# zhaihongjia/SplatLoc

Measured on AMD Instinct MI355X. Metric: fwd+bwd frames/s @1080p, 500k Gaussians, 32 feat-ch; HBM GB/s vs roofline, higher is better.
Workload: dtype f32

## Files before the change

### splatloc_amd/csrc/binning.hip

```cpp
#include "tile_order.h"
#include "composite_common.h"

namespace sr {

__device__ __forceinline__ int f2i_sat_b(float v)
{
    if (!(v > -1.0e9f)) v = -1.0e9f;
    if (!(v < 1.0e9f)) v = 1.0e9f;
    return (int)v;
}

constexpr int EMIT_BLOCK = 256;
constexpr int EMIT_IPT = 4;
static_assert(EMIT_SPAN == EMIT_BLOCK * EMIT_IPT, "common.h: EMIT_SPAN");

template <typename KeyT>
__global__ void __launch_bounds__(EMIT_BLOCK)
emit_kernel(int64_t R, int P , int Pv , int tiles_per_view, int W, int H,
            const uint32_t* __restrict__ offsets,
            const uint32_t* __restrict__ depth_order, const float4* __restrict__ rec,
            KeyT* __restrict__ keys, uint32_t* __restrict__ vals,
            const uint32_t* __restrict__ span_owner ,
            uint32_t* __restrict__ ranges, uint32_t nranges )
{
    for (uint32_t w = blockIdx.x * blockDim.x + threadIdx.x; w < nranges; w += gridDim.x * blockDim.x) ranges[w] = 0u;
    __shared__ uint32_t s_off[EMIT_SPAN + 1];
    __shared__ uint32_t s_gid[EMIT_SPAN], s_org[EMIT_SPAN], s_w[EMIT_SPAN];
    __shared__ int s_min;
    const int t = threadIdx.x;
    const int64_t j0 = (int64_t)blockIdx.x * EMIT_SPAN;
    const uint32_t j0u = (uint32_t)j0;
    int lo = 0, hi = P;
    if (span_owner && blockIdx.x < SPAN_OWNER_CAP) {
        lo = (int)span_owner[blockIdx.x];
        hi = lo + 1;
    }
    while (hi - lo > 1) {
        const int n = hi - lo;
        const int step = (n + EMIT_BLOCK - 1) / EMIT_BLOCK;
        if (t == 0) s_min = EMIT_BLOCK;
        __syncthreads();
        const int last = lo + (t + 1) * step - 1;
        if (last >= hi - 1 || offsets[last] > j0u) atomicMin(&s_min, t);
        __syncthreads();
        const int seg = s_min;
        __syncthreads();
        lo = lo + seg * step;
        hi = min(hi, lo + step);
    }
    const int r_lo = lo;
    for (int q = t; q <= EMIT_SPAN; q += EMIT_BLOCK) {
        const int r = r_lo - 1 + q;
        s_off[q] = r < 0 ? 0u : offsets[min(r, P - 1)];
    }
    __syncthreads();
    const int gx = (W + TILE - 1) / TILE, gy = (H + TILE - 1) / TILE;
    const uint32_t j_last = (uint32_t)(min(R, j0 + (int64_t)EMIT_SPAN) - 1);
    int nr;
    {
        int a = 1, b = EMIT_SPAN + 1;
        while (a < b) {
            const int mid = (a + b) >> 1;
            if (s_off[mid] > j_last) b = mid; else a = mid + 1;
        }
        nr = a;
    }
    for (int q = t; q < nr; q += EMIT_BLOCK) {
        const uint32_t g = depth_order[r_lo + q] & 0xFFFFFFu;
        const float4 p = rec[2 * g];
        const float rf = p.w;
        const int rminx = min(gx, max(0, f2i_sat_b((p.x - rf) / (float)TILE)));
        const int rminy = min(gy, max(0, f2i_sat_b((p.y - rf) / (float)TILE)));
        const int rmaxx = min(gx, max(0, f2i_sat_b((p.x + rf + (float)(TILE - 1)) / (float)TILE)));
        s_gid[q] = g;
        const uint32_t v = (P == Pv) ? 0u : g / (uint32_t)Pv;
        s_org[q] = v * (uint32_t)tiles_per_view + (uint32_t)rminy * (uint32_t)gx + (uint32_t)rminx;
        s_w[q] = (uint32_t)(rmaxx - rminx);
    }
    __syncthreads();
#pragma unroll
    for (int it = 0; it < EMIT_IPT; ++it) {
        const int64_t j = j0 + it * EMIT_BLOCK + t;
        if (j < R) {
            const uint32_t ju = (uint32_t)j;
            int a = 1, b = nr + 1;
            while (a < b) {
                const int mid = (a + b) >> 1;
                if (s_off[mid] > ju) b = mid; else a = mid + 1;
            }
            const uint32_t k = ju - s_off[a - 1];
            const uint32_t w = s_w[a - 1];
            const uint32_t row = k / w;
            keys[j] = (KeyT)(s_org[a - 1] + row * (uint32_t)gx + (k - row * w));
            vals[j] = s_gid[a - 1];
        }
    }
}

int launch_emit(const FramePlan& p, int64_t R, const GeomView& g, uint32_t* keys, uint32_t* vals, uint32_t* ranges,
                uint32_t nranges, hipStream_t stream, bool keys16)
{
    if (R == 0) return SPLATRASTER_OK;
    const int64_t blocks = (R + EMIT_SPAN - 1) / EMIT_SPAN;
    const int n = p.P * p.V;
    const uint32_t* owner = scan_state_bytes(n) ? g.span_owner : nullptr;
    if (keys16)
        hipLaunchKernelGGL(emit_kernel<uint16_t>, dim3((unsigned)blocks), dim3(EMIT_BLOCK), 0, stream, R, n, p.P, p.tiles, p.W, p.H,
                           g.offsets, g.depth_order, g.rec, reinterpret_cast<uint16_t*>(keys), vals, owner, ranges, nranges);
    else
        hipLaunchKernelGGL(emit_kernel<uint32_t>, dim3((unsigned)blocks), dim3(EMIT_BLOCK), 0, stream, R, n, p.P, p.tiles, p.W, p.H,
                           g.offsets, g.depth_order, g.rec, keys, vals, owner, ranges, nranges);
    SR_LAUNCH_CHECK();
    return SPLATRASTER_OK;
}

int launch_ranges_clear(int32_t tiles, uint32_t* ranges, hipStream_t stream)
{
    SR_HIP_CHECK(hipMemsetAsync(ranges, 0, sizeof(uint32_t) * 2 * (size_t)tiles, stream));
    return SPLATRASTER_OK;
}

#ifndef SR_PAYLOAD_NT_MIN
#define SR_PAYLOAD_NT_MIN (8ll << 20)
#endif
static int64_t g_payload_stream_min = SR_PAYLOAD_NT_MIN;
void set_payload_stream_min(int64_t instances) { g_payload_stream_min = instances < 0 ? (int64_t)SR_PAYLOAD_NT_MIN : instances; }

template <bool NT>
__global__ void __launch_bounds__(256)
payload_kernel(int64_t R, int gx, int tiles_per_view, int V, const uint32_t* __restrict__ point_list,
               const uint32_t* __restrict__ tile_list, const float4* __restrict__ rec,
               float4* __restrict__ irec, uint32_t* __restrict__ ipack, uint32_t* __restrict__ ranges)
{
    const int64_t j = (int64_t)blockIdx.x * blockDim.x + threadIdx.x;
    if (j >= R) return;
    const uint32_t g = point_list[j], t = tile_list[j];
    const float4 a0 = rec[2 * (size_t)g], a1 = rec[2 * (size_t)g + 1];
    uint32_t tl = t;
#pragma unroll 1
    for (int v = 1; v < V && tl >= (uint32_t)tiles_per_view; ++v) tl -= (uint32_t)tiles_per_view;
    const uint32_t ty = tl / (uint32_t)gx, tx = tl - ty * (uint32_t)gx;
    const float4 c1 = payload_conic(a1);
    const uint32_t m = g | (quadrant_reach_mask(a0, a1, (float)(tx * TILE), (float)(ty * TILE)) << 24);
    if (NT) {
        typedef float f32x4_t __attribute__((ext_vector_type(4)));
        f32x4_t* out = reinterpret_cast<f32x4_t*>(irec) + 2 * j;
        __builtin_nontemporal_store((f32x4_t){a0.x, a0.y, a0.z, a0.w}, out);
        __builtin_nontemporal_store((f32x4_t){c1.x, c1.y, c1.z, c1.w}, out + 1);
        __builtin_nontemporal_store(m, ipack + j);
    } else {
        irec[2 * j] = a0;
        irec[2 * j + 1] = c1;
        ipack[j] = m;
    }
    if (j == 0 || tile_list[j - 1] != t) ranges[2 * t] = (uint32_t)j;
    if (j == R - 1 || tile_list[j + 1] != t) ranges[2 * t + 1] = (uint32_t)(j + 1);
}

int launch_payload(const FramePlan& p, int64_t R, const GeomView& g, const BinView& b, hipStream_t stream)
{
    if (R == 0) return SPLATRASTER_OK;
    if (R >= g_payload_stream_min)
        hipLaunchKernelGGL(payload_kernel<true>, dim3((unsigned)((R + 255) / 256)), dim3(256), 0, stream, R, p.gx, p.tiles, p.V,
                           b.point_list, b.tile_list, g.rec, b.irec, b.ipack, b.ranges);
    else
        hipLaunchKernelGGL(payload_kernel<false>, dim3((unsigned)((R + 255) / 256)), dim3(256), 0, stream, R, p.gx, p.tiles, p.V,
                           b.point_list, b.tile_list, g.rec, b.irec, b.ipack, b.ranges);
    SR_LAUNCH_CHECK();
    return SPLATRASTER_OK;
}

__global__ void __launch_bounds__(256)
ranges_kernel(int64_t R, const uint32_t* __restrict__ tile_list, uint32_t* __restrict__ ranges)
{
    const int64_t j = (int64_t)blockIdx.x * blockDim.x + threadIdx.x;
    if (j >= R) return;
    const uint32_t t = tile_list[j];
    if (j == 0 || tile_list[j - 1] != t) ranges[2 * t] = (uint32_t)j;
    if (j == R - 1 || tile_list[j + 1] != t) ranges[2 * t + 1] = (uint32_t)(j + 1);
}

template <bool NT>
__global__ void __launch_bounds__(256)
payload_tile_kernel(int gx, int tiles_per_view, const uint32_t* __restrict__ ranges, const uint32_t* __restrict__ point_list,
                    const float4* __restrict__ rec, float4* __restrict__ irec, uint32_t* __restrict__ ipack,
                    uint32_t* __restrict__ cranges)
{
    __shared__ uint32_t s_live[4];
    const uint32_t gt = blockIdx.x;
    const uint32_t beg = ranges[2 * gt], end = ranges[2 * gt + 1];
    const uint32_t tl = gt % (uint32_t)tiles_per_view;
    const uint32_t ty = tl / (uint32_t)gx, tx = tl - ty * (uint32_t)gx;
    const float ox = (float)(tx * TILE), oy = (float)(ty * TILE);
    const int lane = threadIdx.x & (WAVE - 1);
    const int wave = __builtin_amdgcn_readfirstlane((int)(threadIdx.x >> 6));
    const uint64_t lt_mask = (lane == 0) ? 0ull : (~0ull >> (WAVE - lane));
    uint32_t running = 0;
#pragma unroll 1
    for (uint32_t base = beg; base < end; base += 256u) {
        const uint32_t j = base + threadIdx.x;
        uint32_t g = 0u, mask = 0u;
        float4 a0 = make_float4(0.f, 0.f, 0.f, 0.f), a1 = a0;
        if (j < end) {
            g = point_list[j];
            a0 = rec[2 * (size_t)g];
            a1 = rec[2 * (size_t)g + 1];
            mask = quadrant_reach_mask(a0, a1, ox, oy);
        }
        const bool live = mask != 0u;
        const uint64_t ballot = __builtin_amdgcn_ballot_w64(live);
        if (lane == 0) s_live[wave] = (uint32_t)__popcll(ballot);
        __syncthreads();
        const uint32_t n0 = s_live[0], n1 = s_live[1], n2 = s_live[2], n3 = s_live[3];
        __syncthreads();
        const uint32_t before = (wave > 0 ? n0 : 0u) + (wave > 1 ? n1 : 0u) + (wave > 2 ? n2 : 0u);
        if (live) {
            const size_t pos = (size_t)beg + running + before + (uint32_t)__popcll(ballot & lt_mask);
            const float4 c1 = payload_conic(a1);
            const float back = __uint_as_float(j - beg + 1u);
            const uint32_t m = g | (mask << 24);
            if (NT) {
                typedef float f32x4_t __attribute__((ext_vector_type(4)));
                f32x4_t* out = reinterpret_cast<f32x4_t*>(irec) + 2 * pos;
                __builtin_nontemporal_store((f32x4_t){a0.x, a0.y, a0.z, back}, out);
                __builtin_nontemporal_store((f32x4_t){c1.x, c1.y, c1.z, c1.w}, out + 1);
                __builtin_nontemporal_store(m, ipack + pos);
            } else {
                irec[2 * pos] = make_float4(a0.x, a0.y, a0.z, back);
                irec[2 * pos + 1] = c1;
                ipack[pos] = m;
            }
        }
        running += n0 + n1 + n2 + n3;
    }
    if (threadIdx.x == 0) {
        cranges[2 * gt] = beg;
        cranges[2 * gt + 1] = beg + running;
    }
}

int launch_payload_compact(const FramePlan& p, int64_t R, const GeomView& g, const BinView& b, uint32_t* cranges, hipStream_t stream)
{
    const unsigned lists = (unsigned)p.gtiles;
    if (R > 0) {
        hipLaunchKernelGGL(ranges_kernel, dim3((unsigned)((R + 255) / 256)), dim3(256), 0, stream, R, b.tile_list, b.ranges);
        SR_LAUNCH_CHECK();
    }
    if (R >= g_payload_stream_min)
        hipLaunchKernelGGL(payload_tile_kernel<true>, dim3(lists), dim3(256), 0, stream, p.gx, p.tiles, b.ranges, b.point_list, g.rec,
                           b.irec, b.ipack, cranges);
    else
        hipLaunchKernelGGL(payload_tile_kernel<false>, dim3(lists), dim3(256), 0, stream, p.gx, p.tiles, b.ranges, b.point_list, g.rec,
                           b.irec, b.ipack, cranges);
    SR_LAUNCH_CHECK();
    return SPLATRASTER_OK;
}

__global__ void __launch_bounds__(ORDER_THREADS)
tile_order_kernel(int T, const uint32_t* __restrict__ ranges, uint32_t* __restrict__ order, uint32_t* __restrict__ nparts)
{
    __shared__ uint32_t s_cnt[ORDER_BUCKETS];
    __shared__ uint32_t s_wsum[ORDER_THREADS / WAVE];
    tile_order_block(T, [&](int i) { return ranges[2 * i + 1] - ranges[2 * i]; }, order, s_cnt, s_wsum, nparts);
}

int launch_tile_order(const FramePlan& p, const BinView& b, hipStream_t stream)
{
    if (!p.order) return SPLATRASTER_OK;
    hipLaunchKernelGGL(tile_order_kernel, dim3(1), dim3(ORDER_THREADS), 0, stream, (int)p.gtiles, b.ranges, b.tile_order, b.nparts);
    SR_LAUNCH_CHECK();
    return SPLATRASTER_OK;
}

__global__ void __launch_bounds__(256)
pad_features_kernel(int64_t n4 , int C, int PPR, const float* __restrict__ feat,
                    float4* __restrict__ featp4)
{
    const int64_t e = (int64_t)blockIdx.x * blockDim.x + threadIdx.x;
    if (e >= n4) return;
    const int64_t row = e / PPR;
    const int c = (int)(e - row * PPR) * 4;
    const float* src = feat + row * C + c;
    float4 v;
    v.x = src[0];
    v.y = c + 1 < C ? src[1] : 0.0f;
    v.z = c + 2 < C ? src[2] : 0.0f;
    v.w = c + 3 < C ? src[3] : 0.0f;
    featp4[e] = v;
}

int launch_pad_features(int32_t P, int C, const float* feat, float* featp, hipStream_t stream)
{
    const int CP = padded_channels(C);
    const int64_t n4 = (int64_t)P * CP / 4;
    if (n4 == 0 || CP == C) return SPLATRASTER_OK;
    hipLaunchKernelGGL(pad_features_kernel, dim3((unsigned)((n4 + 255) / 256)), dim3(256), 0, stream, n4, C, CP / 4,
                       feat, reinterpret_cast<float4*>(featp));
    SR_LAUNCH_CHECK();
    return SPLATRASTER_OK;
}

}
```

Measured before the change: 766.6.

## Replace emit binary search with owner scan; vectorize ranges and pair rec loads

In the emit kernel, each span start marks its owning Gaussian in shared memory, and a wave-level max-scan with a carry across iterations propagates the owner to every slot. This replaces the per-element binary search, and the integer divide is swapped for a float reciprocal with a correction step. The ranges kernel now handles four tile ids per thread using aligned uint4 loads with a head offset. The payload compaction kernel has lane pairs fetch the two halves of two records and exchange them through DPP quad permutes, so each load instruction is coalesced. These changes add extra shared memory, synchronisation and tricky edge handling, which brings some correctness risk.

```diff
diff --git a/splatloc_amd/csrc/binning.hip b/splatloc_amd/csrc/binning.hip
--- a/splatloc_amd/csrc/binning.hip
+++ b/splatloc_amd/csrc/binning.hip
@@ -26,6 +26,8 @@
     for (uint32_t w = blockIdx.x * blockDim.x + threadIdx.x; w < nranges; w += gridDim.x * blockDim.x) ranges[w] = 0u;
     __shared__ uint32_t s_off[EMIT_SPAN + 1];
     __shared__ uint32_t s_gid[EMIT_SPAN], s_org[EMIT_SPAN], s_w[EMIT_SPAN];
+    __shared__ __attribute__((aligned(8))) uint16_t s_own[EMIT_SPAN];
+    __shared__ uint32_t s_wown[EMIT_BLOCK / WAVE];
     __shared__ int s_min;
     const int t = threadIdx.x;
     const int64_t j0 = (int64_t)blockIdx.x * EMIT_SPAN;
@@ -53,6 +55,7 @@
         const int r = r_lo - 1 + q;
         s_off[q] = r < 0 ? 0u : offsets[min(r, P - 1)];
     }
+    reinterpret_cast<uint2*>(s_own)[t] = make_uint2(0u, 0u);
     __syncthreads();
     const int gx = (W + TILE - 1) / TILE, gy = (H + TILE - 1) / TILE;
     const uint32_t j_last = (uint32_t)(min(R, j0 + (int64_t)EMIT_SPAN) - 1);
@@ -76,23 +79,42 @@
         const uint32_t v = (P == Pv) ? 0u : g / (uint32_t)Pv;
         s_org[q] = v * (uint32_t)tiles_per_view + (uint32_t)rminy * (uint32_t)gx + (uint32_t)rminx;
         s_w[q] = (uint32_t)(rmaxx - rminx);
+        if (q >= 1 && s_off[q + 1] > s_off[q]) s_own[s_off[q] - j0u] = (uint16_t)q;
     }
     __syncthreads();
+    {
+        const int lane = t & (WAVE - 1);
+        const uint2 ow = reinterpret_cast<const uint2*>(s_own)[t];
+        const uint32_t m0 = ow.x & 0xFFFFu, m1 = max(m0, ow.x >> 16), m2 = max(m1, ow.y & 0xFFFFu), m3 = max(m2, ow.y >> 16);
+        uint32_t incl = m3;
+#pragma unroll
+        for (int d = 1; d < WAVE; d <<= 1) {
+            const uint32_t up = (uint32_t)__shfl_up((int)incl, d, WAVE);
+            if (lane >= d) incl = max(incl, up);
+        }
+        uint32_t excl = (uint32_t)__shfl_up((int)incl, 1, WAVE);
+        if (lane == 0) excl = 0u;
+        if (lane == WAVE - 1) s_wown[t / WAVE] = incl;
+        reinterpret_cast<uint2*>(s_own)[t] = make_uint2(max(m0, excl) | max(m1, excl) << 16, max(m2, excl) | max(m3, excl) << 16);
+    }
+    __syncthreads();
+    uint32_t carry = 0u;
+    static_assert(WAVE * EMIT_IPT == EMIT_BLOCK && EMIT_BLOCK / WAVE == EMIT_IPT, "emit_kernel: a wave scans the slots of one iteration");
 #pragma unroll
     for (int it = 0; it < EMIT_IPT; ++it) {
         const int64_t j = j0 + it * EMIT_BLOCK + t;
+        const uint32_t a = max((uint32_t)s_own[it * EMIT_BLOCK + t], carry);
+        carry = max(carry, s_wown[it]);
         if (j < R) {
             const uint32_t ju = (uint32_t)j;
-            int a = 1, b = nr + 1;
-            while (a < b) {
-                const int mid = (a + b) >> 1;
-                if (s_off[mid] > ju) b = mid; else a = mid + 1;
-            }
-            const uint32_t k = ju - s_off[a - 1];
-            const uint32_t w = s_w[a - 1];
-            const uint32_t row = k / w;
-            keys[j] = (KeyT)(s_org[a - 1] + row * (uint32_t)gx + (k - row * w));
-            vals[j] = s_gid[a - 1];
+            const uint32_t k = ju - s_off[a];
+            const uint32_t w = s_w[a];
+            uint32_t row = (uint32_t)((float)k * __frcp_rn((float)w));
+            int col = (int)(k - row * w);
+            if (col < 0) { row -= 1u; col += (int)w; }
+            else if (col >= (int)w) { row += 1u; col -= (int)w; }
+            keys[j] = (KeyT)(s_org[a] + row * (uint32_t)gx + (uint32_t)col);
+            vals[j] = s_gid[a];
         }
     }
 }
@@ -171,13 +193,41 @@
 }
 
 __global__ void __launch_bounds__(256)
-ranges_kernel(int64_t R, const uint32_t* __restrict__ tile_list, uint32_t* __restrict__ ranges)
-{
-    const int64_t j = (int64_t)blockIdx.x * blockDim.x + threadIdx.x;
-    if (j >= R) return;
-    const uint32_t t = tile_list[j];
-    if (j == 0 || tile_list[j - 1] != t) ranges[2 * t] = (uint32_t)j;
-    if (j == R - 1 || tile_list[j + 1] != t) ranges[2 * t + 1] = (uint32_t)(j + 1);
+ranges_kernel(int64_t R, int head, const uint32_t* __restrict__ tile_list, uint32_t* __restrict__ ranges)
+{
+    const int64_t j0 = ((int64_t)blockIdx.x * blockDim.x + threadIdx.x) * 4 - head;
+    if (j0 >= R) return;
+    uint32_t t[6];
+    if (j0 >= 0 && j0 + 4 <= R) {
+        const uint4 q = *reinterpret_cast<const uint4*>(tile_list + j0);
+        t[1] = q.x; t[2] = q.y; t[3] = q.z; t[4] = q.w;
+        t[0] = j0 > 0 ? tile_list[j0 - 1] : 0u;
+        t[5] = j0 + 4 < R ? tile_list[j0 + 4] : 0u;
+    } else {
+#pragma unroll
+        for (int e = 0; e < 6; ++e) {
+            const int64_t j = j0 - 1 + e;
+            t[e] = (j >= 0 && j < R) ? tile_list[j] : 0u;
+        }
+    }
+#pragma unroll
+    for (int e = 1; e <= 4; ++e) {
+        const int64_t j = j0 - 1 + e;
+        if (j < 0 || j >= R) continue;
+        if (j == 0 || t[e - 1] != t[e]) ranges[2 * t[e]] = (uint32_t)j;
+        if (j == R - 1 || t[e + 1] != t[e]) ranges[2 * t[e] + 1] = (uint32_t)(j + 1);
+    }
+}
+
+template <int CTRL>
+__device__ __forceinline__ uint32_t quad_perm_u32(uint32_t v)
+{
+    return (uint32_t)__builtin_amdgcn_update_dpp(0, (int)v, CTRL, 0xf, 0xf, false);
+}
+__device__ __forceinline__ float4 quad_perm_f4(const float4& v)
+{
+    return make_float4(__uint_as_float(quad_perm_u32<0xB1>(__float_as_uint(v.x))), __uint_as_float(quad_perm_u32<0xB1>(__float_as_uint(v.y))),
+                       __uint_as_float(quad_perm_u32<0xB1>(__float_as_uint(v.z))), __uint_as_float(quad_perm_u32<0xB1>(__float_as_uint(v.w))));
 }
 
 template <bool NT>
@@ -195,18 +245,19 @@
     const int lane = threadIdx.x & (WAVE - 1);
     const int wave = __builtin_amdgcn_readfirstlane((int)(threadIdx.x >> 6));
     const uint64_t lt_mask = (lane == 0) ? 0ull : (~0ull >> (WAVE - lane));
+    const bool odd = threadIdx.x & 1u;
     uint32_t running = 0;
 #pragma unroll 1
     for (uint32_t base = beg; base < end; base += 256u) {
         const uint32_t j = base + threadIdx.x;
-        uint32_t g = 0u, mask = 0u;
-        float4 a0 = make_float4(0.f, 0.f, 0.f, 0.f), a1 = a0;
-        if (j < end) {
-            g = point_list[j];
-            a0 = rec[2 * (size_t)g];
-            a1 = rec[2 * (size_t)g + 1];
-            mask = quadrant_reach_mask(a0, a1, ox, oy);
-        }
+        const bool valid = j < end;
+        const uint32_t g = point_list[valid ? j : end - 1u];
+        const uint32_t ge = quad_perm_u32<0xA0>(g), go = quad_perm_u32<0xF5>(g);
+        const float4 x = rec[2 * (size_t)ge + odd];
+        const float4 y = rec[2 * (size_t)go + odd];
+        const float4 got = quad_perm_f4(odd ? x : y);
+        const float4 a0 = odd ? got : x, a1 = odd ? y : got;
+        const uint32_t mask = valid ? quadrant_reach_mask(a0, a1, ox, oy) : 0u;
         const bool live = mask != 0u;
         const uint64_t ballot = __builtin_amdgcn_ballot_w64(live);
         if (lane == 0) s_live[wave] = (uint32_t)__popcll(ballot);
@@ -243,7 +294,9 @@
 {
     const unsigned lists = (unsigned)p.gtiles;
     if (R > 0) {
-        hipLaunchKernelGGL(ranges_kernel, dim3((unsigned)((R + 255) / 256)), dim3(256), 0, stream, R, b.tile_list, b.ranges);
+        const int head = (int)((reinterpret_cast<uintptr_t>(b.tile_list) >> 2) & 3u);
+        const int64_t groups = (R + head + 3) / 4;
+        hipLaunchKernelGGL(ranges_kernel, dim3((unsigned)((groups + 255) / 256)), dim3(256), 0, stream, R, head, b.tile_list, b.ranges);
         SR_LAUNCH_CHECK();
     }
     if (R >= g_payload_stream_min)
```

Result: no change. 773.3, median of 6 (+0.9%).

## Replace per-instance binary search in emit with bitmap rank and vectorize binning kernels

Applied to the files above, without the earlier changes.

The emit kernel drops the per-output binary search over staged offsets. It now marks each Gaussian's start slot in a shared bitmap and finds the owner by a wave-level popcount prefix scan. Each thread produces four consecutive keys, using a magic-multiply division, and writes them with vector stores when the pointers are aligned. The ranges kernel now handles four entries per thread with vector loads, and the payload compaction loop processes 512 entries per iteration with prefetched point ids and a double-buffered counter array, halving its barriers. This adds complexity and bit-packing limits on start slots and widths, in exchange for less shared-memory search, fewer divisions and fewer synchronizations.

```diff
diff --git a/splatloc_amd/csrc/binning.hip b/splatloc_amd/csrc/binning.hip
--- a/splatloc_amd/csrc/binning.hip
+++ b/splatloc_amd/csrc/binning.hip
@@ -1,4 +1,5 @@
 #include "tile_order.h"
+#include "tile_div.h"
 #include "composite_common.h"
 
 namespace sr {
@@ -13,8 +14,9 @@
 constexpr int EMIT_BLOCK = 256;
 constexpr int EMIT_IPT = 4;
 static_assert(EMIT_SPAN == EMIT_BLOCK * EMIT_IPT, "common.h: EMIT_SPAN");
-
-template <typename KeyT>
+static_assert(EMIT_SPAN == 1024 && EMIT_BLOCK == 4 * WAVE, "emit_kernel: 32 map words scanned by 32 lanes, start slots of 10 bits");
+
+template <typename KeyT, bool VEC>
 __global__ void __launch_bounds__(EMIT_BLOCK)
 emit_kernel(int64_t R, int P , int Pv , int tiles_per_view, int W, int H,
             const uint32_t* __restrict__ offsets,
@@ -24,9 +26,10 @@
             uint32_t* __restrict__ ranges, uint32_t nranges )
 {
     for (uint32_t w = blockIdx.x * blockDim.x + threadIdx.x; w < nranges; w += gridDim.x * blockDim.x) ranges[w] = 0u;
-    __shared__ uint32_t s_off[EMIT_SPAN + 1];
-    __shared__ uint32_t s_gid[EMIT_SPAN], s_org[EMIT_SPAN], s_w[EMIT_SPAN];
-    __shared__ int s_min;
+    __shared__ uint4 s_rank[EMIT_SPAN];
+    __shared__ uint32_t s_bits[EMIT_SPAN / 32];
+    __shared__ uint32_t s_k0;
+    __shared__ int s_min, s_more;
     const int t = threadIdx.x;
     const int64_t j0 = (int64_t)blockIdx.x * EMIT_SPAN;
     const uint32_t j0u = (uint32_t)j0;
@@ -49,52 +52,106 @@
         hi = min(hi, lo + step);
     }
     const int r_lo = lo;
-    for (int q = t; q <= EMIT_SPAN; q += EMIT_BLOCK) {
-        const int r = r_lo - 1 + q;
-        s_off[q] = r < 0 ? 0u : offsets[min(r, P - 1)];
-    }
-    __syncthreads();
+    const uint32_t j_last = (uint32_t)(min(R, j0 + (int64_t)EMIT_SPAN) - 1);
     const int gx = (W + TILE - 1) / TILE, gy = (H + TILE - 1) / TILE;
-    const uint32_t j_last = (uint32_t)(min(R, j0 + (int64_t)EMIT_SPAN) - 1);
-    int nr;
-    {
-        int a = 1, b = EMIT_SPAN + 1;
-        while (a < b) {
-            const int mid = (a + b) >> 1;
-            if (s_off[mid] > j_last) b = mid; else a = mid + 1;
-        }
-        nr = a;
-    }
-    for (int q = t; q < nr; q += EMIT_BLOCK) {
-        const uint32_t g = depth_order[r_lo + q] & 0xFFFFFFu;
-        const float4 p = rec[2 * g];
+    auto stage = [&](int q, uint32_t o, uint32_t g, const float4& p) {
         const float rf = p.w;
         const int rminx = min(gx, max(0, f2i_sat_b((p.x - rf) / (float)TILE)));
         const int rminy = min(gy, max(0, f2i_sat_b((p.y - rf) / (float)TILE)));
         const int rmaxx = min(gx, max(0, f2i_sat_b((p.x + rf + (float)(TILE - 1)) / (float)TILE)));
-        s_gid[q] = g;
         const uint32_t v = (P == Pv) ? 0u : g / (uint32_t)Pv;
-        s_org[q] = v * (uint32_t)tiles_per_view + (uint32_t)rminy * (uint32_t)gx + (uint32_t)rminx;
-        s_w[q] = (uint32_t)(rmaxx - rminx);
-    }
+        const uint32_t org = v * (uint32_t)tiles_per_view + (uint32_t)rminy * (uint32_t)gx + (uint32_t)rminx;
+        const uint32_t w = (uint32_t)(rmaxx - rminx);
+        const uint32_t start = q == 0 ? 0u : o - j0u;
+        s_rank[q] = make_uint4(g | (start << 24), org, w | ((start >> 8) << 28), tile_div_magic(w));
+        if (q == 0) s_k0 = j0u - o;
+        else atomicOr(&s_bits[start >> 5], 1u << (start & 31u));
+    };
+    uint32_t o0 = offsets[max(0, min(r_lo - 1 + t, P - 1))];
+    const uint32_t g0 = depth_order[min(r_lo + t, P - 1)] & 0xFFFFFFu;
+    if (t < EMIT_SPAN / 32) s_bits[t] = 0u;
+    if (t == 0 && r_lo == 0) o0 = 0u;
+    const bool in0 = o0 <= j_last;
+    if (t == EMIT_BLOCK - 1) s_more = in0;
+    const float4 p0 = rec[in0 ? 2 * (size_t)g0 : (size_t)0];
     __syncthreads();
-#pragma unroll
-    for (int it = 0; it < EMIT_IPT; ++it) {
-        const int64_t j = j0 + it * EMIT_BLOCK + t;
-        if (j < R) {
-            const uint32_t ju = (uint32_t)j;
-            int a = 1, b = nr + 1;
-            while (a < b) {
-                const int mid = (a + b) >> 1;
-                if (s_off[mid] > ju) b = mid; else a = mid + 1;
+    if (in0) stage(t, o0, g0, p0);
+    if (s_more) {
+        uint32_t o[EMIT_IPT], g[EMIT_IPT];
+        float4 p[EMIT_IPT];
+        bool in[EMIT_IPT];
+#pragma unroll
+        for (int i = 1; i < EMIT_IPT; ++i) o[i] = offsets[min(r_lo - 1 + t + i * EMIT_BLOCK, P - 1)];
+#pragma unroll
+        for (int i = 1; i < EMIT_IPT; ++i) g[i] = depth_order[min(r_lo + t + i * EMIT_BLOCK, P - 1)] & 0xFFFFFFu;
+#pragma unroll
+        for (int i = 1; i < EMIT_IPT; ++i) {
+            in[i] = o[i] <= j_last;
+            p[i] = rec[in[i] ? 2 * (size_t)g[i] : (size_t)0];
+        }
+#pragma unroll
+        for (int i = 1; i < EMIT_IPT; ++i) asm volatile("" : "+v"(p[i].x), "+v"(p[i].y), "+v"(p[i].w));
+#pragma unroll
+        for (int i = 1; i < EMIT_IPT; ++i)
+            if (in[i]) stage(t + i * EMIT_BLOCK, o[i], g[i], p[i]);
+    }
+    __syncthreads();
+    const int lane = t & (WAVE - 1);
+    const uint32_t word = s_bits[lane & 31];
+    const uint32_t cnt = (uint32_t)__popc(word);
+    uint32_t inc = cnt;
+#pragma unroll
+    for (int dl = 1; dl < 32; dl <<= 1) {
+        const uint32_t up = (uint32_t)__shfl_up((int)inc, dl, 32);
+        if ((lane & 31) >= dl) inc += up;
+    }
+    const int wi = t >> 3;
+    const uint32_t before = (uint32_t)__shfl((int)(inc - cnt), wi, 32);
+    const uint32_t mine = (uint32_t)__shfl((int)word, wi, 32);
+    const uint32_t sh = 4u * (uint32_t)(t & 7);
+    uint32_t q = before + (uint32_t)__popc(mine & ((1u << sh) - 1u));
+    const uint32_t nib = mine >> sh;
+    const uint32_t k0 = s_k0;
+    uint32_t key[EMIT_IPT], val[EMIT_IPT];
+#pragma unroll
+    for (int e = 0; e < EMIT_IPT; ++e) {
+        q += (nib >> e) & 1u;
+        const uint4 rk = s_rank[q];
+        const uint32_t start = (rk.x >> 24) | ((rk.z >> 28) << 8);
+        const uint32_t w = rk.z & 0x0FFFFFFFu;
+        const uint32_t k = (uint32_t)(4 * t + e) - start + (q == 0u ? k0 : 0u);
+        uint32_t row, col;
+        tile_div(k, w, rk.w, row, col);
+        key[e] = rk.y + row * (uint32_t)gx + col;
+        val[e] = rk.x & 0xFFFFFFu;
+    }
+    const int64_t j = j0 + 4 * t;
+    if (VEC && j + EMIT_IPT <= R) {
+        *reinterpret_cast<uint4*>(vals + j) = make_uint4(val[0], val[1], val[2], val[3]);
+        if (sizeof(KeyT) == 2)
+            *reinterpret_cast<uint2*>(keys + j) = make_uint2(key[0] | (key[1] << 16), key[2] | (key[3] << 16));
+        else
+            *reinterpret_cast<uint4*>(keys + j) = make_uint4(key[0], key[1], key[2], key[3]);
+    } else {
+#pragma unroll
+        for (int e = 0; e < EMIT_IPT; ++e)
+            if (j + e < R) {
+                keys[j + e] = (KeyT)key[e];
+                vals[j + e] = val[e];
             }
-            const uint32_t k = ju - s_off[a - 1];
-            const uint32_t w = s_w[a - 1];
-            const uint32_t row = k / w;
-            keys[j] = (KeyT)(s_org[a - 1] + row * (uint32_t)gx + (k - row * w));
-            vals[j] = s_gid[a - 1];
-        }
-    }
+    }
+}
+
+template <typename KeyT>
+static void launch_emit_as(unsigned blocks, hipStream_t stream, int64_t R, int n, const FramePlan& p, const GeomView& g, KeyT* keys,
+                           uint32_t* vals, const uint32_t* owner, uint32_t* ranges, uint32_t nranges)
+{
+    if ((((uintptr_t)keys | (uintptr_t)vals) & 15u) == 0)
+        hipLaunchKernelGGL((emit_kernel<KeyT, true>), dim3(blocks), dim3(EMIT_BLOCK), 0, stream, R, n, p.P, p.tiles, p.W, p.H,
+                           g.offsets, g.depth_order, g.rec, keys, vals, owner, ranges, nranges);
+    else
+        hipLaunchKernelGGL((emit_kernel<KeyT, false>), dim3(blocks), dim3(EMIT_BLOCK), 0, stream, R, n, p.P, p.tiles, p.W, p.H,
+                           g.offsets, g.depth_order, g.rec, keys, vals, owner, ranges, nranges);
 }
 
 int launch_emit(const FramePlan& p, int64_t R, const GeomView& g, uint32_t* keys, uint32_t* vals, uint32_t* ranges,
@@ -105,11 +162,9 @@
     const int n = p.P * p.V;
     const uint32_t* owner = scan_state_bytes(n) ? g.span_owner : nullptr;
     if (keys16)
-        hipLaunchKernelGGL(emit_kernel<uint16_t>, dim3((unsigned)blocks), dim3(EMIT_BLOCK), 0, stream, R, n, p.P, p.tiles, p.W, p.H,
-                           g.offsets, g.depth_order, g.rec, reinterpret_cast<uint16_t*>(keys), vals, owner, ranges, nranges);
+        launch_emit_as((unsigned)blocks, stream, R, n, p, g, reinterpret_cast<uint16_t*>(keys), vals, owner, ranges, nranges);
     else
-        hipLaunchKernelGGL(emit_kernel<uint32_t>, dim3((unsigned)blocks), dim3(EMIT_BLOCK), 0, stream, R, n, p.P, p.tiles, p.W, p.H,
-                           g.offsets, g.depth_order, g.rec, keys, vals, owner, ranges, nranges);
+        launch_emit_as((unsigned)blocks, stream, R, n, p, g, keys, vals, owner, ranges, nranges);
     SR_LAUNCH_CHECK();
     return SPLATRASTER_OK;
 }
@@ -170,23 +225,64 @@
     return SPLATRASTER_OK;
 }
 
+template <bool NT>
+__device__ __forceinline__ void payload_store(bool live, size_t pos, const float4& a0, const float4& a1, uint32_t g, uint32_t mask,
+                                              uint32_t back_bits, float4* __restrict__ irec, uint32_t* __restrict__ ipack)
+{
+    if (!live) return;
+    const float4 c1 = payload_conic(a1);
+    const float back = __uint_as_float(back_bits);
+    const uint32_t m = g | (mask << 24);
+    if (NT) {
+        typedef float f32x4_t __attribute__((ext_vector_type(4)));
+        f32x4_t* out = reinterpret_cast<f32x4_t*>(irec) + 2 * pos;
+        __builtin_nontemporal_store((f32x4_t){a0.x, a0.y, a0.z, back}, out);
+        __builtin_nontemporal_store((f32x4_t){c1.x, c1.y, c1.z, c1.w}, out + 1);
+        __builtin_nontemporal_store(m, ipack + pos);
+    } else {
+        irec[2 * pos] = make_float4(a0.x, a0.y, a0.z, back);
+        irec[2 * pos + 1] = c1;
+        ipack[pos] = m;
+    }
+}
+
+constexpr int RANGES_EPT = 4;
+template <bool VEC>
 __global__ void __launch_bounds__(256)
 ranges_kernel(int64_t R, const uint32_t* __restrict__ tile_list, uint32_t* __restrict__ ranges)
 {
-    const int64_t j = (int64_t)blockIdx.x * blockDim.x + threadIdx.x;
+    const int64_t j = RANGES_EPT * ((int64_t)blockIdx.x * blockDim.x + threadIdx.x);
     if (j >= R) return;
-    const uint32_t t = tile_list[j];
-    if (j == 0 || tile_list[j - 1] != t) ranges[2 * t] = (uint32_t)j;
-    if (j == R - 1 || tile_list[j + 1] != t) ranges[2 * t + 1] = (uint32_t)(j + 1);
-}
-
+    const int n = (int)min((int64_t)RANGES_EPT, R - j);
+    uint32_t t[RANGES_EPT + 2];
+    if (VEC && n == RANGES_EPT) {
+        const uint4 v = *reinterpret_cast<const uint4*>(tile_list + j);
+        t[1] = v.x; t[2] = v.y; t[3] = v.z; t[4] = v.w;
+    } else {
+#pragma unroll
+        for (int e = 0; e < RANGES_EPT; ++e) t[1 + e] = tile_list[min(j + e, R - 1)];
+    }
+    const bool first = j == 0, last = j + n == R;
+    t[0] = first ? 0u : tile_list[j - 1];
+    t[RANGES_EPT + 1] = last ? 0u : tile_list[j + RANGES_EPT];
+#pragma unroll
+    for (int e = 0; e < RANGES_EPT; ++e) {
+        if (e < n) {
+            const uint32_t c = t[1 + e];
+            if ((first && e == 0) || t[e] != c) ranges[2 * c] = (uint32_t)(j + e);
+            if ((last && e == n - 1) || t[e + 2] != c) ranges[2 * c + 1] = (uint32_t)(j + e + 1);
+        }
+    }
+}
+
+constexpr uint32_t PAYLOAD_STEP = 512;
 template <bool NT>
 __global__ void __launch_bounds__(256)
 payload_tile_kernel(int gx, int tiles_per_view, const uint32_t* __restrict__ ranges, const uint32_t* __restrict__ point_list,
                     const float4* __restrict__ rec, float4* __restrict__ irec, uint32_t* __restrict__ ipack,
                     uint32_t* __restrict__ cranges)
 {
-    __shared__ uint32_t s_live[4];
+    __shared__ uint32_t s_live[2][8];
     const uint32_t gt = blockIdx.x;
     const uint32_t beg = ranges[2 * gt], end = ranges[2 * gt + 1];
     const uint32_t tl = gt % (uint32_t)tiles_per_view;
@@ -196,42 +292,45 @@
     const int wave = __builtin_amdgcn_readfirstlane((int)(threadIdx.x >> 6));
     const uint64_t lt_mask = (lane == 0) ? 0ull : (~0ull >> (WAVE - lane));
     uint32_t running = 0;
+    if (beg < end) {
+        uint32_t g0 = point_list[min(beg + threadIdx.x, end - 1u)], g1 = point_list[min(beg + threadIdx.x + 256u, end - 1u)];
+        int buf = 0;
 #pragma unroll 1
-    for (uint32_t base = beg; base < end; base += 256u) {
-        const uint32_t j = base + threadIdx.x;
-        uint32_t g = 0u, mask = 0u;
-        float4 a0 = make_float4(0.f, 0.f, 0.f, 0.f), a1 = a0;
-        if (j < end) {
-            g = point_list[j];
-            a0 = rec[2 * (size_t)g];
-            a1 = rec[2 * (size_t)g + 1];
-            mask = quadrant_reach_mask(a0, a1, ox, oy);
+        for (uint32_t base = beg; base < end; base += PAYLOAD_STEP, buf ^= 1) {
+            const uint32_t j0 = base + threadIdx.x, j1 = j0 + 256u;
+            const float4 a00 = rec[2 * (size_t)g0], a01 = rec[2 * (size_t)g0 + 1];
+            const float4 a10 = rec[2 * (size_t)g1], a11 = rec[2 * (size_t)g1 + 1];
+            const uint32_t h0 = g0, h1 = g1;
+            const uint32_t mask0 = j0 < end ? quadrant_reach_mask(a00, a01, ox, oy) : 0u;
+            const uint32_t mask1 = j1 < end ? quadrant_reach_mask(a10, a11, ox, oy) : 0u;
+            const bool live0 = mask0 != 0u, live1 = mask1 != 0u;
+            const uint64_t ballot0 = __builtin_amdgcn_ballot_w64(live0), ballot1 = __builtin_amdgcn_ballot_w64(live1);
+            if (base + PAYLOAD_STEP < end) {
+                g0 = point_list[min(j0 + PAYLOAD_STEP, end - 1u)];
+                g1 = point_list[min(j1 + PAYLOAD_STEP, end - 1u)];
+            }
+            if (lane == 0) {
+                s_live[buf][wave] = (uint32_t)__popcll(ballot0);
+                s_live[buf][4 + wave] = (uint32_t)__popcll(ballot1);
+            }
+            __syncthreads();
+            uint32_t n[8];
+#pragma unroll
+            for (int c = 0; c < 8; ++c) n[c] = s_live[buf][c];
+            uint32_t before0 = 0u, all = 0u;
+#pragma unroll
+            for (int c = 0; c < 8; ++c) {
+                before0 += c < wave ? n[c] : 0u;
+                all += n[c];
+            }
+            uint32_t before1 = n[0] + n[1] + n[2] + n[3];
+#pragma unroll
+            for (int c = 0; c < 4; ++c) before1 += c < wave ? n[4 + c] : 0u;
+            const size_t first = (size_t)beg + running;
+            payload_store<NT>(live0, first + before0 + (uint32_t)__popcll(ballot0 & lt_mask), a00, a01, h0, mask0, j0 - beg + 1u, irec, ipack);
+            payload_store<NT>(live1, first + before1 + (uint32_t)__popcll(ballot1 & lt_mask), a10, a11, h1, mask1, j1 - beg + 1u, irec, ipack);
+            running += all;
         }
-        const bool live = mask != 0u;
-        const uint64_t ballot = __builtin_amdgcn_ballot_w64(live);
-        if (lane == 0) s_live[wave] = (uint32_t)__popcll(ballot);
-        __syncthreads();
-        const uint32_t n0 = s_live[0], n1 = s_live[1], n2 = s_live[2], n3 = s_live[3];
-        __syncthreads();
-        const uint32_t before = (wave > 0 ? n0 : 0u) + (wave > 1 ? n1 : 0u) + (wave > 2 ? n2 : 0u);
-        if (live) {
-            const size_t pos = (size_t)beg + running + before + (uint32_t)__popcll(ballot & lt_mask);
-            const float4 c1 = payload_conic(a1);
-            const float back = __uint_as_float(j - beg + 1u);
-            const uint32_t m = g | (mask << 24);
-            if (NT) {
-                typedef float f32x4_t __attribute__((ext_vector_type(4)));
-                f32x4_t* out = reinterpret_cast<f32x4_t*>(irec) + 2 * pos;
-                __builtin_nontemporal_store((f32x4_t){a0.x, a0.y, a0.z, back}, out);
-                __builtin_nontemporal_store((f32x4_t){c1.x, c1.y, c1.z, c1.w}, out + 1);
-                __builtin_nontemporal_store(m, ipack + pos);
-            } else {
-                irec[2 * pos] = make_float4(a0.x, a0.y, a0.z, back);
-                irec[2 * pos + 1] = c1;
-                ipack[pos] = m;
-            }
-        }
-        running += n0 + n1 + n2 + n3;
     }
     if (threadIdx.x == 0) {
         cranges[2 * gt] = beg;
@@ -243,7 +342,11 @@
 {
     const unsigned lists = (unsigned)p.gtiles;
     if (R > 0) {
-        hipLaunchKernelGGL(ranges_kernel, dim3((unsigned)((R + 255) / 256)), dim3(256), 0, stream, R, b.tile_list, b.ranges);
+        const unsigned blocks = (unsigned)((R + 256 * RANGES_EPT - 1) / (256 * RANGES_EPT));
+        if (((uintptr_t)b.tile_list & 15u) == 0)
+            hipLaunchKernelGGL(ranges_kernel<true>, dim3(blocks), dim3(256), 0, stream, R, b.tile_list, b.ranges);
+        else
+            hipLaunchKernelGGL(ranges_kernel<false>, dim3(blocks), dim3(256), 0, stream, R, b.tile_list, b.ranges);
         SR_LAUNCH_CHECK();
     }
     if (R >= g_payload_stream_min)
diff --git a/splatloc_amd/csrc/tile_div.h b/splatloc_amd/csrc/tile_div.h
--- /dev/null
+++ b/splatloc_amd/csrc/tile_div.h
@@ -0,0 +1,20 @@
+#pragma once
+#include <stdint.h>
+
+namespace sr {
+
+__host__ __device__ __forceinline__ uint32_t tile_div_magic(uint32_t w) { return 0xFFFFFFFFu / (w ? w : 1u); }
+
+__device__ __forceinline__ void tile_div(uint32_t k, uint32_t w, uint32_t m, uint32_t& row, uint32_t& col)
+{
+    uint32_t q = __umulhi(k, m);
+    uint32_t r = k - q * w;
+    if (r >= w) {
+        r -= w;
+        ++q;
+    }
+    row = q;
+    col = r;
+}
+
+}
```

Result: no change. 779.2 before, 783.8 after (median of 6 runs) (+0.6%).
